# JingwenWang95/DSP-SLAM

Measured on NVIDIA H100. Metric: object-recons/sec (2048 pts, 10 GN iters), higher is better.
Workload: dtype f16x3-split (fp32 accumulate)

## Files before the change

### dsp_slam_b200/csrc/dspgn_api.cu

```cuda
#include <cuda_runtime.h>
#include <cstdio>
#include <cstring>
#include <cmath>
#include <string>
#include <vector>
#include <new>
#include <algorithm>
#include <atomic>

#include <cub/device/device_scan.cuh>

#include "dspgn_common.cuh"
#include "dspgn_simt.cuh"
#include "dspgn_solve.cuh"
#include "dspgn_tc.cuh"
#include "dspgn_mesh.cuh"
#include "dspgn_frame.cuh"
#include "dspgn_mono.cuh"

using namespace dspgn;

namespace {

constexpr int kEvCap = 1 << 18;
// ... 75 lines not shown
  DevBuf d_q_flag, d_q_ctr, d_tiles_left, d_obj_iter;
  int* d_tbase_static = nullptr;
  int* d_tbase_r_static = nullptr;
  DevBuf d_run;
  HostBuf h_run;
  cudaEvent_t ev_run_upload = nullptr;
  bool run_upload_pending = false;
  bool run_table_valid = false;
  bool run_table_gated = false;
  int total_tiles128 = 0;
  long long total_ray_tiles128 = 0;
  int max_tiles128 = 0;
  bool mega_enabled = true;
  bool compact_rays = true;
  DevBuf d_ev, d_seg, d_ln, d_vpre;
  bool events_on = false;
  HostBuf h_results;
  DspgnCounters ctr{};
  bool timing = false;
  std::vector<cudaEvent_t> ev;
  size_t ev_used = 0;
  std::vector<cudaEvent_t> ev_solve;
  size_t evs_used = 0;
  cudaEvent_t ev_run0 = nullptr, ev_run1 = nullptr;
  cudaStream_t stream2 = nullptr;
  cudaEvent_t ev_fork = nullptr, ev_join = nullptr;
  cudaEvent_t ev_upload = nullptr;
  bool upload_pending = false;
  bool mega_ran = false;
  bool band_rows_pending = false;
// ... 239 lines not shown
  int eng = cfg->engine;
  if (eng == DSPGN_ENGINE_AUTO) {
    const char* e = getenv("DSPGN_ENGINE");
    if (e && !strcmp(e, "simt")) eng = DSPGN_ENGINE_SIMT;
    else if (e && !strcmp(e, "tc")) eng = DSPGN_ENGINE_TC;
    else eng = (tc_ok && tc_engine_default()) ? DSPGN_ENGINE_TC : DSPGN_ENGINE_SIMT;
  }
  if (eng == DSPGN_ENGINE_TC && !tc_ok) { dspgn_solver_destroy(s); return fail(DSPGN_E_ARG, "tensor-core engine unavailable for this decoder shape"); }
  s->engine = eng;
  CU(cudaFuncSetAttribute(k_decoder_simt, cudaFuncAttributeMaxDynamicSharedMemorySize, (int)sizeof(SimtSmem)));
  for (auto* d : s->classes)
    if (d->has_ln) {
      if (s->d_ln.reserve(4 * (size_t)s->num_sms * DSPGN_MAX_LINEAR * kHid * kTP)) { dspgn_solver_destroy(s); return fail(DSPGN_E_ALLOC, "cudaMalloc"); }
      break;
    }
  if (int rc = tc_setup_kernels(g_err)) { dspgn_solver_destroy(s); return rc; }
  if (const char* m = getenv("DSPGN_MEGA")) s->mega_enabled = (m[0] != '0');
  if (const char* m = getenv("DSPGN_COMPACT_RAYS")) s->compact_rays = (m[0] != '0');
  if (cfg->schedule == DSPGN_SCHED_LAUNCHES) s->mega_enabled = false;
  else if (cfg->schedule == DSPGN_SCHED_PERSISTENT) s->mega_enabled = true;
  else if (cfg->schedule != DSPGN_SCHED_AUTO) { dspgn_solver_destroy(s); return fail(DSPGN_E_ARG, "bad schedule"); }
  s->events_on = getenv("DSPGN_CLK") != nullptr;
  CU(cudaEventCreateWithFlags(&s->ev_upload, cudaEventDisableTiming));
  CU(cudaEventCreateWithFlags(&s->ev_run_upload, cudaEventDisableTiming));
  CU(cudaStreamCreateWithFlags(&s->stream2, cudaStreamNonBlocking));
  CU(cudaEventCreateWithFlags(&s->ev_fork, cudaEventDisableTiming));
  CU(cudaEventCreateWithFlags(&s->ev_join, cudaEventDisableTiming));
  CU(cudaEventCreate(&s->ev_run0));
  CU(cudaEventCreate(&s->ev_run1));
#undef CU
// ... 3 lines not shown
    if (e_ != cudaSuccess)                                                                \
      return fail(DSPGN_E_CUDA, std::string(#call) + ": " + cudaGetErrorString(e_));      \
  } while (0)
  *out = s;
  return 0;
}

void dspgn_solver_destroy(DspgnSolver* s) {
  if (!s) return;
  cudaSetDevice(s->device);
  cudaDeviceSynchronize();
  s->flight.active = false;
  dspgn_gather_close(s);
  for (DevBuf* b : {&s->d_decs, &s->d_stage, &s->d_state, &s->d_part_s, &s->d_part_r, &s->d_tbase, &s->d_V, &s->d_m, &s->d_results, &s->d_active,
                    &s->d_sdf, &s->d_bx, &s->d_bs, &s->d_br, &s->d_dbg, &s->d_q_flag, &s->d_q_ctr,
                    &s->d_tiles_left, &s->d_obj_iter, &s->d_ev, &s->d_seg, &s->d_ln, &s->d_vpre, &s->d_run,
                    &s->d_grid_pts, &s->d_mgrid, &s->d_mws, &s->d_mscan_tmp, &s->d_mout, &s->d_mesh_sel}) b->release();
  s->h_stage.release();
  s->h_mbase.release();
  s->h_results.release();
  s->h_run.release();
  s->h_mesh_sel.release();
  s->h_flight.release();
  if (s->ev_flight) cudaEventDestroy(s->ev_flight);
  for (auto e : s->ev) cudaEventDestroy(e);
  for (auto e : s->ev_solve) cudaEventDestroy(e);
  if (s->ev_upload) cudaEventDestroy(s->ev_upload);
  if (s->ev_run_upload) cudaEventDestroy(s->ev_run_upload);
  if (s->ev_fork) cudaEventDestroy(s->ev_fork);
  if (s->ev_join) cudaEventDestroy(s->ev_join);
  if (s->stream2) cudaStreamDestroy(s->stream2);
// ... 426 lines not shown
    MegaArgs q;
    if (int rc = mega_args(s, p, q)) return rc;
    CU(cudaMemsetAsync(q.q_flag, 0, 4 * (size_t)q.q_cap, s->stream));
    if (int rc = launch_init(s, b, p, q)) return rc;
    TermArgs a = base_term(s, MODE_SDF);
    a.huber_b = s->cfg.b2;
    a.huber_b1 = s->cfg.b1;
    a.tile_base = s->d_tbase_static;
    a.part_r = s->d_part_r.as<float>(); a.tile_base_r = s->d_tbase_r_static;
    if (p.any[DSPGN_MODE_POSE] && p.iters[DSPGN_MODE_POSE] > 5) { a.pt_active = s->d_active.as<uint8_t>(); a.cut_iter = 4; }
    if (q.log.ev) CU(cudaMemsetAsync(q.log.ev, 0, 8, s->stream));
    SolveArgs v = base_solve(s);
    v.base_s = s->d_tbase_static; v.base_r = s->d_tbase_r_static; v.tile_rows = kTcRows; v.iter_index = 0;
    const int grid = grid_sms(s);
    if (s->timing) cudaEventRecord(next_event(s), s->stream);
    if (render) k_gn_persistent_render<<<grid, kTcThreads, kTcSmemBytes, s->stream>>>(b, a, q, v);
    else k_gn_persistent<<<grid, kTcThreads, kTcSmemBytes, s->stream>>>(b, a, q, v);
    if (s->timing) cudaEventRecord(next_event(s), s->stream);
    s->ctr.kernel_launches += 1;
    for (int m = 0; m < 2; ++m) s->ctr.rows_fwd_bwd += p.pts[m] * p.iters[m];
    s->band_rows_pending = render;
    s->mega_ran = true;
    CU(cudaGetLastError());
    CU(cudaEventRecord(s->ev_run1, s->stream));
    return 0;
  }
  if (int rc = launch_init(s, b, p)) return rc;
  auto iterate = [&](const RunPlan& pl, int n_iters) -> int {
    for (int e = 0; e < n_iters; ++e) {
      if (int rc = launch_terms(s, b, pl, e)) return rc;
      SolveArgs v = base_solve(s);
      v.iter_index = e;
// ... 1393 lines not shown
```

### dsp_slam_b200/csrc/dspgn_tc.cuh

```cuda
#pragma once
#include <cuda_fp16.h>
#include <string>
#include <vector>
#include "dspgn_simt.cuh"
#include "dspgn_solve.cuh"

namespace dspgn {

constexpr int kTcThreads = 384;
constexpr int kTcEpiThreads = 256;
constexpr int kTcStages = 4;
constexpr int kTcStageBytes = 16384;
constexpr int kTcAloBytes = 32768;
constexpr int kTcProducerRegs = 40, kTcConsumerRegs = 232;
static_assert(128 * kTcProducerRegs + 256 * kTcConsumerRegs <= 384 * 168, "setmaxnreg budget exceeds the CTA's registers");

__host__ __device__ constexpr int tc_mma_n(int n) { return n <= 80 ? 80 : (n <= 192 ? 192 : 256); }
__host__ __device__ constexpr int tc_pad_k_steps(int k_steps) { return (k_steps + 3) / 4 * 4; }

__device__ __forceinline__ uint32_t smem_u32(const void* p) { return (uint32_t)__cvta_generic_to_shared(p); }

__device__ __forceinline__ void mbar_init(uint64_t* bar, uint32_t count) {
  asm volatile("mbarrier.init.shared::cta.b64 [%0], %1;" ::"r"(smem_u32(bar)), "r"(count) : "memory");
}
__device__ __forceinline__ void mbar_arrive(uint32_t bar) {
  asm volatile("mbarrier.arrive.shared::cta.b64 _, [%0];" ::"r"(bar) : "memory");
}
// ... 6 lines not shown
      ".reg .pred p;\n\t"
      "WAIT_LOOP:\n\t"
      "mbarrier.try_wait.parity.shared::cta.b64 p, [%0], %1;\n\t"
      "@p bra DONE;\n\t"
      "bra WAIT_LOOP;\n\t"
      "DONE:\n\t"
      "}" ::"r"(bar), "r"(parity) : "memory");
}
__device__ __forceinline__ void mbar_wait(uint64_t* bar, uint32_t parity) { mbar_wait(smem_u32(bar), parity); }
__device__ __forceinline__ void fence_barrier_init() { asm volatile("fence.mbarrier_init.release.cluster;" ::: "memory"); }

__device__ __forceinline__ void bulk_g2s(void* smem_dst, const void* gmem_src, uint32_t bytes, uint64_t* bar) {
  asm volatile("cp.async.bulk.shared::cluster.global.mbarrier::complete_tx::bytes [%0], [%1], %2, [%3];" ::"r"(smem_u32(smem_dst)),
               "l"(gmem_src), "r"(bytes), "r"(smem_u32(bar)) : "memory");
}

__device__ __forceinline__ void fence_proxy_async() { asm volatile("fence.proxy.async.shared::cta;" ::: "memory"); }
__device__ __forceinline__ void wg_fence() { asm volatile("wgmma.fence.sync.aligned;" ::: "memory"); }
__device__ __forceinline__ void wg_commit() { asm volatile("wgmma.commit_group.sync.aligned;" ::: "memory"); }
__device__ __forceinline__ void wg_wait0() { asm volatile("wgmma.wait_group.sync.aligned 0;" ::: "memory"); }
__device__ __forceinline__ void wg_wait1() { asm volatile("wgmma.wait_group.sync.aligned 1;" ::: "memory"); }
template <int REGS> __device__ __forceinline__ void setmaxnreg_inc() { asm volatile("setmaxnreg.inc.sync.aligned.u32 %0;" ::"n"(REGS)); }
template <int REGS> __device__ __forceinline__ void setmaxnreg_dec() { asm volatile("setmaxnreg.dec.sync.aligned.u32 %0;" ::"n"(REGS)); }
__device__ __forceinline__ void wg_bar_sync(int g) { asm volatile("bar.sync %0, 128;" ::"r"(3 + g) : "memory"); }

#define DSPGN_D8(o) "+f"(d[o + 0]), "+f"(d[o + 1]), "+f"(d[o + 2]), "+f"(d[o + 3]), "+f"(d[o + 4]), "+f"(d[o + 5]), "+f"(d[o + 6]), "+f"(d[o + 7])
#define DSPGN_D128                                                                                                    \
  DSPGN_D8(0), DSPGN_D8(8), DSPGN_D8(16), DSPGN_D8(24), DSPGN_D8(32), DSPGN_D8(40), DSPGN_D8(48), DSPGN_D8(56),         \
      DSPGN_D8(64), DSPGN_D8(72), DSPGN_D8(80), DSPGN_D8(88), DSPGN_D8(96), DSPGN_D8(104), DSPGN_D8(112), DSPGN_D8(120)
#define DSPGN_D96                                                                                                     \
// ... 70 lines not shown
  d |= (uint64_t)1 << 16;
  d |= (uint64_t)32 << 32;
  d |= (uint64_t)2 << 62;
  return d;
}

__device__ __forceinline__ void split_pack(float a, float b, uint32_t& hi, uint32_t& lo) {
  __half2 h = __floats2half2_rn(a, b);
  float2 back = __half22float2(h);
  __half2 l = __floats2half2_rn(a - back.x, b - back.y);
  hi = *reinterpret_cast<uint32_t*>(&h);
  lo = *reinterpret_cast<uint32_t*>(&l);
}

constexpr int kJpStride = 76;
struct TcSmemTail {
  float Jp[kTcRows * kJpStride];
  uint32_t maskw[8 * 4 * kTcEpiThreads];
  float bias[9 * kHid];
  float wlast[kHid];
  float w0x[3 * kHid];
  float zs[kMaxCode + 16];
  float xr[3 * kTcRows];
  float rr[kTcRows], rsc[kTcRows];
  float yrow[kTcRows], scr[kTcRows];
  int prefix[kMaxObjScan + 1];
  int warp_tmp[32];
  uint64_t w_full[kTcStages], w_empty[kTcStages];
  int cur_class;
  int fifo[4]; int fifo_pub; int epi_seq; int last_flag;
  TcPlan plans[DSPGN_MAX_CLASSES];
  BatchDev ctx_b; MegaArgs ctx_q; SolveArgs ctx_sv;
  int push_base, push_nF, push_nS, push_o;
  float ost[16]; int ost_rows;
};
constexpr size_t kTcSmemBytes = 1024 + (size_t)kTcStages * kTcStageBytes + 2 * (size_t)kTcAloBytes + sizeof(TcSmemTail);
static_assert(kTcSmemBytes <= 227 * 1024, "tensor-core engine shared memory exceeds the 227 KB per block of sm_90");
static_assert(offsetof(TcSmemTail, bias) % 8 == 0 && offsetof(TcSmemTail, w0x) % 8 == 0,
              "the SDF-tile epilogues read bias and W0 column pairs as float2");

__device__ __forceinline__ int frag_col(int e, int q) { return 8 * (e >> 2) + 2 * q + (e & 1); }
__device__ __forceinline__ int opaque_int(int v) {
  int r;
  asm volatile("mov.b32 %0, %1;" : "=r"(r) : "r"(v));
  return r;
}

__device__ __forceinline__ void store_operand(const float (&v)[128], uint32_t (&ah)[64], unsigned char* alo, int rl, int q, int grp,
                                              int pslot = -1) {
  DSPGN_PROBE_T(ts);
#pragma unroll
  for (int t = 0; t < 16; ++t) {
#pragma unroll
    for (int h = 0; h < 4; ++h) {
// ... 146 lines not shown
      float w = hy ? bj.y : bj.x;
      w = fmaf(hy ? w0.y : w0.x, hb ? xb0 : xa0, w);
      w = fmaf(hy ? w1.y : w1.x, hb ? xb1 : xa1, w);
      w = fmaf(hy ? w2.y : w2.x, hb ? xb2 : xa2, w);
      mw[e >> 5] |= (w > 0.f ? 1u : 0u) << (e & 31);
      acc[e] = w > 0.f ? w : 0.f;
    }
  }
}

__device__ __forceinline__ void release_stage(uint32_t w_empty, int s) {
  __syncwarp();
  if ((threadIdx.x & 31) == 0) mbar_arrive(w_empty + 8u * s);
}

template <int N>
__device__ __forceinline__ void wg_gemm(float (&acc)[128], const uint32_t (&ah)[64], uint32_t alo, uint32_t ring,
                                        uint32_t bars, uint32_t& phase, int nch) {
  static_assert(kTcStages == 4, "one ring lap per K chunk");
  const uint32_t w_full = bars, w_empty = bars + 8u * kTcStages;
#pragma unroll
  for (int i = 0; i < 128; ++i) acc[i] = 0.f;
#pragma unroll
  for (int c = 0; c < 4; ++c) {
    if (c < nch) {
      const uint32_t ph = phase ^ (uint32_t)(c & 1);
#pragma unroll
      for (int s = 0; s < kTcStages; ++s) {
        DSPGN_PROBE_T(tf);
        mbar_wait(w_full + 8u * s, ph);
        DSPGN_PROBE_ADD(PR_WFULL, tf);
        wg_fence();
        const uint32_t bw = ring + (uint32_t)s * kTcStageBytes;
#pragma unroll
        for (int k = 0; k < 2; ++k) {
          const int t = 4 * c + 2 * (s & 1) + k;
          const uint64_t bd = make_desc_w(bw + 32u * k);
          Wgmma<N>::rs(acc, ah[4 * t], ah[4 * t + 1], ah[4 * t + 2], ah[4 * t + 3], bd);
          if (s < 2) Wgmma<N>::ss(acc, make_desc(alo + 8192u * c + 32u * (t & 3)), bd);
        }
        wg_commit();
        if (s == 1) {
          DSPGN_PROBE_T(tw);
          wg_wait1();
          DSPGN_PROBE_ADD(PR_WGWAIT, tw);
          release_stage(w_empty, 0);
          if (c > 0) release_stage(w_empty, 3);
        } else if (s == 3) {
          DSPGN_PROBE_T(tw);
          wg_wait1();
          DSPGN_PROBE_ADD(PR_WGWAIT, tw);
          release_stage(w_empty, 1);
          release_stage(w_empty, 2);
        }
      }
    }
  }
  DSPGN_PROBE_T(tw);
  wg_wait0();
  DSPGN_PROBE_ADD(PR_WGWAIT, tw);
  release_stage(w_empty, 3);
  phase ^= (uint32_t)(nch & 1);
}

__device__ __forceinline__ void produce_step(const unsigned char* src, int nch, uint32_t img_bytes, unsigned char* ring,
                                             uint64_t* w_full, uint64_t* w_empty, uint32_t& phase) {
  for (int c = 0; c < nch; ++c) {
    for (int s = 0; s < kTcStages; ++s) {
      DSPGN_PROBE_T(te);
      mbar_wait(&w_empty[s], phase ^ 1);
      DSPGN_PROBE_ADD(PR_WEMPTY, te);
      mbar_expect_tx(&w_full[s], img_bytes);
      bulk_g2s(ring + (size_t)s * kTcStageBytes, src + (size_t)(kTcStages * c + s) * img_bytes, img_bytes, &w_full[s]);
    }
    phase ^= 1;
  }
}

struct TileRef { int o, row0, slot, mode, tile; };

constexpr unsigned long long kMegaTimeoutNs = 30ull * 1000ull * 1000ull * 1000ull;
__device__ inline int mega_pop(const MegaArgs& q, int n_obj) {
  for (;;) {
    const int t = atomicAdd(&q.ctr->head, 1);
    if (t >= q.q_cap) return -1;
    unsigned long long t0 = 0;
    int item = kItemNop;
    for (unsigned spins = 0;; ++spins) {
      const int v = ldv(q.q_flag + t);
      if (v != 0) { __threadfence(); item = v - 1; break; }
      if (ldv(&q.ctr->done_objects) >= n_obj || ldv(&q.ctr->abort_flag) != 0) return -1;
      __nanosleep(256);
      if ((spins & 1023u) == 1023u) {
        const unsigned long long now = globaltimer_ns();
        if (t0 == 0) t0 = now;
        else if (now - t0 > kMegaTimeoutNs) { atomicExch(&q.ctr->abort_flag, 1); return -1; }
      }
    }
    if (item != kItemNop) return item;
  }
}

template <int SCHED>
__device__ __forceinline__ bool tile_at(const BatchDev& b, const TermArgs& a, TcSmemTail& S, int seq, int total_tiles, TileRef& t) {
  constexpr bool MEGA = SCHED != 0;
  if (!MEGA) {
    const int tile = blockIdx.x + seq * gridDim.x;
    if (tile >= total_tiles) return false;
    t.o = find_object(S.prefix, b.n_obj, tile);
    t.tile = tile - S.prefix[t.o];
    t.row0 = t.tile * kTcRows;
    t.slot = tile;
    t.mode = a.mode;
    return true;
  } else {
    volatile int* pub = &S.fifo_pub;
    while (*pub <= seq) __nanosleep(64);
    const int item = reinterpret_cast<volatile int*>(S.fifo)[seq & 3];
    if (item < 0) return false;
// ... 9 lines not shown

__device__ __forceinline__ int mega_rows(const BatchDev& b, const MegaArgs& q, const ObjMeta& M, int o, int mode) {
  if (mode == MODE_SDF) return M.n_pts;
  if (mode == MODE_BAND) return ldv(b.band_m + o);
  if (q.vpre != nullptr) return ldv(q.vpre + vpre_base(M, o) + M.n_rays) >> 7;
  return M.n_rays * b.D;
}

__device__ inline void mega_push(const MegaArgs& q, int kind, int o, int n) {
  if (n <= 0) return;
  const int base = atomicAdd(&q.ctr->tail, n);
  __threadfence();
  for (int j = 0; j < n; ++j) *reinterpret_cast<volatile int*>(q.q_flag + base + j) = make_item(kind, o, j) + 1;
}

__device__ __noinline__ void mega_solve_and_advance(TcSmemTail& S, int o, int tid) {
  const BatchDev& b = S.ctx_b;
  const MegaArgs& q = S.ctx_q;
  const SolveArgs& sv = S.ctx_sv;
  __threadfence();
  SolveSmem& SM = *reinterpret_cast<SolveSmem*>(S.Jp);
  const int it = ldv(q.obj_iter + o);
  const bool render = q.render && b.state[o].mode == DSPGN_MODE_JOINT;
  if (tid == 0) log_event(q.log, ev_desc(EV_SOLVE_BEGIN, 0, o, it));
  const int fin = solve_object<true>(b, sv, q.log, o, tid, SM, it + 1 >= b.state[o].n_iter);
  epi_bar_sync();
  int vh = -1;
  if (!fin && render && q.vpre != nullptr) {
    const ObjMeta M = b.meta[o];
    if (M.n_rays > 0) vh = valid_sample_ranges<true>(M, b.state[o], b.rays, b.D, q.vpre + vpre_base(M, o), tid, kTcEpiThreads, S.warp_tmp);
  }
// ... 23 lines not shown
    S.push_base = base;
  }
  epi_bar_sync();
  const int base = S.push_base;
  if (base >= 0) {
    const int nF = S.push_nF, n = nF + S.push_nS;
    const int po = S.push_o;
    __threadfence();
    epi_bar_sync();
    for (int j = tid; j < n; j += kTcEpiThreads)
      *reinterpret_cast<volatile int*>(q.q_flag + base + j) = ((j < nF) ? make_item(MODE_RAYFWD, po, j) : make_item(MODE_SDF, po, j - nF)) + 1;
  }
}

template <int SCHED>
__device__ __forceinline__ void tc_body(const BatchDev& b, const TermArgs& a, const MegaArgs& q, const SolveArgs& sv) {
  constexpr bool MEGA = SCHED != 0;
  constexpr bool RENDER = SCHED == 2;
  extern __shared__ unsigned char tc_smem_raw[];
  unsigned char* ring = tc_smem_raw + ((1024u - (smem_u32(tc_smem_raw) & 1023u)) & 1023u);
  TcSmemTail& S = *reinterpret_cast<TcSmemTail*>(ring + (size_t)kTcStages * kTcStageBytes + 2 * (size_t)kTcAloBytes);
  const int tid = threadIdx.x, warp = tid >> 5, lane = tid & 31;

  const int total_tiles = MEGA ? 0 : build_tile_prefix(b, a, kTcRows, S.prefix, S.warp_tmp);
  {
    const int nwords = b.n_classes * (int)(sizeof(TcPlan) / 4);
    for (int i = tid; i < nwords; i += kTcThreads) {
      const int c = i / (int)(sizeof(TcPlan) / 4), w = i % (int)(sizeof(TcPlan) / 4);
      reinterpret_cast<int*>(&S.plans[c])[w] = reinterpret_cast<const int*>(&b.decs[c].tc_plan)[w];
    }
  }
  if (tid == 0) {
    for (int i = 0; i < kTcStages; ++i) { mbar_init(&S.w_full[i], 1); mbar_init(&S.w_empty[i], 8); }
    S.cur_class = -1;
    S.fifo_pub = 0; S.epi_seq = 0; S.last_flag = 0;
    if (MEGA) { S.ctx_b = b; S.ctx_q = q; S.ctx_sv = sv; }
    fence_barrier_init();
  }
  __syncthreads();

  if (warp >= 8) {
    setmaxnreg_dec<kTcProducerRegs>();
    if (warp == 8 && lane == 0) {
      uint32_t phase = 0;
      DSPGN_PROBE_T(tloop);
      for (int seq = 0;; ++seq) {
        if (MEGA) {
          DSPGN_PROBE_T(tp);
          volatile int* es = &S.epi_seq;
          while (seq - *es >= 3) __nanosleep(64);
          const int item = mega_pop(q, b.n_obj);
          DSPGN_PROBE_ADD(PR_POP, tp);
          if (item >= 0) log_event(q.log, ev_desc(EV_POPPED, item >> kItemKindShift, (item >> kItemObjShift) & kItemObjMask, item & kItemTileMask));
          reinterpret_cast<volatile int*>(S.fifo)[seq & 3] = item;
          __threadfence_block();
          *reinterpret_cast<volatile int*>(&S.fifo_pub) = seq + 1;
        }
        TileRef tr;
        if (!tile_at<SCHED>(b, a, S, seq, total_tiles, tr)) break;
        const int o = tr.o;
        const int cls = b.meta[o].class_id;
        const TcPlan& plan = S.plans[cls];
        const unsigned char* blob = b.decs[cls].tc_blob;
        const bool fwd_only = (tr.mode == MODE_RAYFWD || tr.mode == MODE_PTSFWD || (!MEGA && tr.mode == MODE_GRIDFWD));
        const int ns = (RENDER && tr.mode == kKindScan) ? 0 : (fwd_only ? plan.n_fwd : plan.n_steps);
        for (int s = 0; s < ns; ++s)
          produce_step(blob + plan.step[s].w_off, plan.step[s].k_steps / 4, 64u * (uint32_t)plan.step[s].n_mma, ring, S.w_full,
                       S.w_empty, phase);
      }
      DSPGN_PROBE_ADD(PR_PROD_LOOP, tloop);
    }
  } else {
    setmaxnreg_inc<kTcConsumerRegs>();
    const int grp = warp >> 2;
    const int r = tid & 127;
    const int qd = lane & 3;
    const int rl = 16 * (warp & 3) + (lane >> 2);
    const int rowA = 64 * grp + rl, rowB = rowA + 8;
    unsigned char* const alo = ring + (size_t)kTcStages * kTcStageBytes + (size_t)grp * kTcAloBytes;
    const uint32_t alo_s = smem_u32(alo), ring_s = smem_u32(ring);
    uint32_t phase = 0;
    float acc[128];
    uint32_t ah[64];
    DSPGN_PROBE_T(tloop);
    for (int seq = 0;; ++seq) {
      TileRef tr;
      DSPGN_PROBE_T(tq);
      if (!tile_at<SCHED>(b, a, S, seq, total_tiles, tr)) break;
      DSPGN_PROBE_ADD(PR_FIFO, tq);
      DSPGN_PROBE_T(tpro);
      if (MEGA && tid == 0) { *reinterpret_cast<volatile int*>(&S.epi_seq) = seq + 1; log_event(q.log, ev_desc(EV_TILE_BEGIN, tr.mode, tr.o, tr.tile)); }
      if (RENDER && tr.mode == kKindScan) {
        const int o = tr.o;
        scan_chunk(b, sv.prm.th, q.vpre, q.seg_cnt, o, tr.tile, tid);
        __threadfence();
        epi_bar_sync();
// ... 109 lines not shown
          xform_point(Toc, __fmul_rn(rq[0], d), __fmul_rn(rq[1], d), __fmul_rn(rq[2], d), x0, x1, x2);
          sc = inside_unit_sphere(x0, x1, x2) ? 1.f : 0.f;
        }
      }
      if (grp == 0) { S.xr[r] = x0; S.xr[kTcRows + r] = x1; S.xr[2 * kTcRows + r] = x2; S.scr[r] = sc; }
      epi_bar_sync();
      DSPGN_PROBE_ADD(PR_PRO_GLOBAL, tpro);
      DSPGN_PROBE_T(tl0);
      if (tid == 0) S.cur_class = M.class_id;

      auto inp = [&](int i, int row) -> float {
        const int j = i - L;
        return (j < 0) ? S.zs[i] : ((unsigned)j < 3u ? S.xr[j * kTcRows + row] : 0.f);
      };
      uint32_t* const maskw = S.maskw + tid;
      auto put_operand = [&](int pslot) {
        if (SCHED == 1) store_operand_stsm(acc, ah, alo_s, grp, pslot);
        else store_operand(acc, ah, alo, rl, qd, grp, pslot);
      };

      {
        const int kk = plan.step[0].k_steps * 16;
        const int n0out = dec.out_dim[0];
        const float* w0x = S.w0x;
        const float xa0 = S.xr[rowA], xa1 = S.xr[kTcRows + rowA], xa2 = S.xr[2 * kTcRows + rowA];
        const float xb0 = S.xr[rowB], xb1 = S.xr[kTcRows + rowB], xb2 = S.xr[2 * kTcRows + rowB];
        const int qs = opaque_int(qd);
        uint32_t mw[4] = {0u, 0u, 0u, 0u};
        if (SCHED == 1 && kk == kHid && n0out == kHid) {
          epi_layer0_256(acc, mw, S.bias, w0x, qs, xa0, xa1, xa2, xb0, xb1, xb2);
        } else {
#pragma unroll
          for (int e = 0; e < 128; ++e) {
            const int c = frag_col(e, qs);
            const bool hb = (e & 2) != 0;
            float w = S.bias[c];
            w = fmaf(w0x[c], hb ? xb0 : xa0, w);
            w = fmaf(w0x[kHid + c], hb ? xb1 : xa1, w);
            w = fmaf(w0x[2 * kHid + c], hb ? xb2 : xa2, w);
            const bool on = (c < kk) && (c < n0out) && (w > 0.f);
            mw[e >> 5] |= (on ? 1u : 0u) << (e & 31);
            acc[e] = on ? w : 0.f;
          }
        }
#pragma unroll
        for (int w = 0; w < 4; ++w) maskw[w * kTcEpiThreads] = mw[w];
        put_operand(-1);
      }
      DSPGN_PROBE_ADD(PR_PRO_L0, tl0);
      DSPGN_PROBE_ADD(PR_PROLOGUE, tpro);
      DSPGN_PROBE_COUNT(PR_TILES);

      float yv = 0.f;
      for (int s = 0; s < ns; ++s) {
        const TcStep st = plan.step[s];
        const bool more = (s + 1 < ns);
        const int k_next = more ? plan.step[s + 1].k_steps * 16 : 0;
        const int nm = st.n_mma;
        if (MEGA && tid == 0 && s == 0) log_event(q.log, ev_desc(EV_FIRST_MMA, tr.mode, tr.o, tr.tile));
        const int nch = st.k_steps / 4;
        DSPGN_PROBE_T(tg);
        if (nm == 80) wg_gemm<80>(acc, ah, alo_s, ring_s, smem_u32(S.w_full), phase, nch);
        else if (nm == 192) wg_gemm<192>(acc, ah, alo_s, ring_s, smem_u32(S.w_full), phase, nch);
        else wg_gemm<256>(acc, ah, alo_s, ring_s, smem_u32(S.w_full), phase, nch);
        DSPGN_PROBE_ADD(PR_GEMM, tg);
        DSPGN_PROBE_T(tepi);
        wg_bar_sync(grp);
        DSPGN_PROBE_ADD(PR_EPI_ENTRY, tepi);
        DSPGN_PROBE_T(tval);
#ifdef DSPGN_STALL_PROBE
        const int pk = PR_EPI_KIND + 3 * (st.kind == TK_FWD_PENULT ? EK_PENULT
                                          : st.kind == TK_FWD_HIDDEN ? (st.cat_off >= 0 ? EK_FWD_CAT : EK_FWD)
                                          : st.kind == TK_BWD_MID ? (st.cat_off >= 0 ? EK_BWD_SKIP : EK_BWD) : EK_BWD_FIRST);
#else
        constexpr int pk = -1;
#endif
        const int qs = opaque_int(qd);

        if (st.kind == TK_FWD_PENULT) {
          const float* bb = S.bias + st.layer * kHid;
          float pa = 0.f, pb = 0.f;
          uint32_t mw[4] = {0u, 0u, 0u, 0u};
#pragma unroll
          for (int e = 0; e < 128; ++e) {
            const int c = frag_col(e, qs);
            if (c < nm) {
              const float w = acc[e] + bb[c];
              mw[e >> 5] |= (w > 0.f ? 1u : 0u) << (e & 31);
              if (e & 2) pb = fmaf(fmaxf(w, 0.f), S.wlast[c], pb);
              else pa = fmaf(fmaxf(w, 0.f), S.wlast[c], pa);
            }
          }
#pragma unroll
          for (int w = 0; w < 4; ++w) maskw[(4 * st.layer + w) * kTcEpiThreads] = mw[w];
          pa += __shfl_xor_sync(0xffffffffu, pa, 1);
          pb += __shfl_xor_sync(0xffffffffu, pb, 1);
          pa += __shfl_xor_sync(0xffffffffu, pa, 2);
          pb += __shfl_xor_sync(0xffffffffu, pb, 2);
          const float blast = S.bias[(st.layer + 1) * kHid];
          const float ya = tanhf(pa + blast), yb = tanhf(pb + blast);
          if (qd == 0) { S.yrow[rowA] = ya; S.yrow[rowB] = yb; }
          epi_bar_sync();
          yv = S.yrow[r];
          if (fwd_only) {
            if (grp == 0 && r < nrows) {
              const size_t base = (mode == MODE_RAYFWD) ? (size_t)M.smp_off
                                  : (grid_mode ? (size_t)a.grid_slot[o] * a.grid_rows : (size_t)M.pts_off);
              b.sdf[base + row0 + r] = (sc != 0.f) ? yv : INFINITY;
            }
// ... 25 lines not shown
            else if (st.cat_off >= 0) epi_concat_input<0, 0>(acc, qs, k_next, st.cat_off, L, S.zs, S.xr, rowA, rowB);
          } else {
#pragma unroll
            for (int e = 0; e < 128; ++e) {
              const int c = frag_col(e, qs);
              float t = 0.f;
              if (c < nm) {
                const float w = acc[e] + bb[c];
                mw[e >> 5] |= (w > 0.f ? 1u : 0u) << (e & 31);
                t = fmaxf(w, 0.f);
              }
              if (st.cat_off >= 0 && c >= st.cat_off) t = inp(c - st.cat_off, (e & 2) ? rowB : rowA);
              acc[e] = (c < k_next) ? t : 0.f;
            }
          }
#pragma unroll
          for (int w = 0; w < 4; ++w) maskw[(4 * st.layer + w) * kTcEpiThreads] = mw[w];
          DSPGN_PROBE_ADD(pk, tval);
          put_operand(pk);
        } else if (st.kind == TK_BWD_MID) {
          uint32_t mw[4];
#pragma unroll
          for (int w = 0; w < 4; ++w) mw[w] = maskw[(4 * st.mask_layer + w) * kTcEpiThreads];
          if (SCHED == 1) {
            if (st.cat_off == 189 && L == 64 && in0 == 67 && nm == kHid) epi_skip_grad<189, 64>(acc, qs, nm, st.cat_off, in0, L, S.Jp, rowA, rowB);
            else if (st.cat_off >= 0) epi_skip_grad<0, 0>(acc, qs, nm, st.cat_off, in0, L, S.Jp, rowA, rowB);
            if (nm == 256 && k_next == 256) epi_bwd_mid<256, 256>(acc, mw, nm, k_next);
            else if (nm == 256 && k_next == 192) epi_bwd_mid<256, 192>(acc, mw, nm, k_next);
            else epi_bwd_mid<0, 0>(acc, mw, nm, k_next);
          } else {
#pragma unroll
            for (int e = 0; e < 128; ++e) {
              const int c = frag_col(e, qs);
              float t = 0.f;
              if (c < nm) {
                const float v = acc[e];
                t = ((mw[e >> 5] >> (e & 31)) & 1u) ? v : 0.f;
                if (st.cat_off >= 0 && c >= st.cat_off) {
// ... 141 lines not shown
        }
        DSPGN_PROBE_ADD(PR_TILE_END, tend);
        if (act == 2) {
          DSPGN_PROBE_T(tsv);
          mega_solve_and_advance(S, o, tid);
          DSPGN_PROBE_ADD(PR_SOLVE, tsv);
          DSPGN_PROBE_COUNT(PR_SOLVES);
        }
      }
    }
    DSPGN_PROBE_ADD(PR_LOOP, tloop);
  }
}

__global__ void __launch_bounds__(kTcThreads, 1) k_decoder_tc(BatchDev b, TermArgs a) {
  tc_body<0>(b, a, MegaArgs{}, SolveArgs{});
}
__global__ void __launch_bounds__(kTcThreads, 1) k_gn_persistent(BatchDev b, TermArgs a, MegaArgs q, SolveArgs sv) {
  tc_body<1>(b, a, q, sv);
}
__global__ void __launch_bounds__(kTcThreads, 1) k_gn_persistent_render(BatchDev b, TermArgs a, MegaArgs q, SolveArgs sv) {
  tc_body<2>(b, a, q, sv);
}

constexpr size_t kTcSelftestSmem = 1024 + (size_t)kTcStages * kTcStageBytes + 2 * (size_t)kTcAloBytes + 64;
__global__ void __launch_bounds__(kTcThreads, 1) k_tc_selftest(const float* __restrict__ A, int lda, const unsigned char* __restrict__ blob,
                                                               int n_mma, int k_steps, float* __restrict__ D) {
  extern __shared__ unsigned char st_raw[];
  unsigned char* ring = st_raw + ((1024u - (smem_u32(st_raw) & 1023u)) & 1023u);
  uint64_t* bars = reinterpret_cast<uint64_t*>(ring + (size_t)kTcStages * kTcStageBytes + 2 * (size_t)kTcAloBytes);
  uint64_t* w_full = bars;
  uint64_t* w_empty = bars + kTcStages;
  const int tid = threadIdx.x, warp = tid >> 5, lane = tid & 31;
  if (tid == 0) {
    for (int i = 0; i < kTcStages; ++i) { mbar_init(&w_full[i], 1); mbar_init(&w_empty[i], 8); }
    fence_barrier_init();
  }
  __syncthreads();
  const int n_img = tc_mma_n(n_mma), nch = tc_pad_k_steps(k_steps) / 4;
  uint32_t phase = 0;
  if (warp >= 8) {
    setmaxnreg_dec<kTcProducerRegs>();
    if (warp == 8 && lane == 0) produce_step(blob, nch, 64u * (uint32_t)n_img, ring, w_full, w_empty, phase);
    return;
  }
  setmaxnreg_inc<kTcConsumerRegs>();
  const int grp = warp >> 2, qd = lane & 3, rl = 16 * (warp & 3) + (lane >> 2);
  const int rowA = 64 * grp + rl, rowB = rowA + 8;
  unsigned char* alo = ring + (size_t)kTcStages * kTcStageBytes + (size_t)grp * kTcAloBytes;
  float acc[128];
  uint32_t ah[64];
#pragma unroll
  for (int e = 0; e < 128; ++e) {
    const int c = frag_col(e, qd);
    acc[e] = (c < k_steps * 16) ? A[(size_t)((e & 2) ? rowB : rowA) * lda + c] : 0.f;
  }
  store_operand(acc, ah, alo, rl, qd, grp);
  if (n_img == 80) wg_gemm<80>(acc, ah, smem_u32(alo), smem_u32(ring), smem_u32(bars), phase, nch);
  else if (n_img == 192) wg_gemm<192>(acc, ah, smem_u32(alo), smem_u32(ring), smem_u32(bars), phase, nch);
  else wg_gemm<256>(acc, ah, smem_u32(alo), smem_u32(ring), smem_u32(bars), phase, nch);
#pragma unroll
  for (int e = 0; e < 128; ++e) {
    const int c = frag_col(e, qd);
    if (c < n_mma) D[(size_t)((e & 2) ? rowB : rowA) * n_mma + c] = acc[e];
  }
}

struct TcDecoderHost {
  bool ok = false;
  void* blob = nullptr;
  size_t blob_bytes = 0;
};

template <class F>
inline void tc_pack_images(std::vector<unsigned char>& out, int n_img, int k_steps, F&& elem) {
// ... 68 lines not shown
  P.n_steps = ns;
  void* d = nullptr;
  if (cudaMalloc(&d, blob.size()) != cudaSuccess) { cudaGetLastError(); err = "cudaMalloc(tc blob)"; return DSPGN_E_ALLOC; }
  if (cudaMemcpy(d, blob.data(), blob.size(), cudaMemcpyHostToDevice) != cudaSuccess) { cudaFree(d); err = "cudaMemcpy(tc blob)"; return DSPGN_E_CUDA; }
  h.blob = d; h.blob_bytes = blob.size(); h.ok = true;
  dv->tc_blob = reinterpret_cast<const unsigned char*>(d);
  return 0;
}

inline void tc_free_decoder(TcDecoderHost& h) {
  if (h.blob) cudaFree(h.blob);
  h.blob = nullptr; h.ok = false;
}

inline int tc_setup_kernels(std::string& err) {
  if (cudaFuncSetAttribute(k_decoder_tc, cudaFuncAttributeMaxDynamicSharedMemorySize, (int)kTcSmemBytes) != cudaSuccess) {
    err = std::string("cudaFuncSetAttribute(k_decoder_tc): ") + cudaGetErrorString(cudaGetLastError());
    return DSPGN_E_CUDA;
  }
  if (cudaFuncSetAttribute(k_gn_persistent, cudaFuncAttributeMaxDynamicSharedMemorySize, (int)kTcSmemBytes) != cudaSuccess ||
      cudaFuncSetAttribute(k_gn_persistent_render, cudaFuncAttributeMaxDynamicSharedMemorySize, (int)kTcSmemBytes) != cudaSuccess) {
    err = std::string("cudaFuncSetAttribute(k_gn_persistent): ") + cudaGetErrorString(cudaGetLastError());
    return DSPGN_E_CUDA;
  }
  if (cudaFuncSetAttribute(k_tc_selftest, cudaFuncAttributeMaxDynamicSharedMemorySize, (int)kTcSelftestSmem) != cudaSuccess) {
    err = std::string("cudaFuncSetAttribute(k_tc_selftest): ") + cudaGetErrorString(cudaGetLastError());
    return DSPGN_E_CUDA;
  }
  return 0;
}

inline bool tc_engine_default() { return true; }

inline int tc_launch_term(const BatchDev& b, const TermArgs& a, int num_sms, long long tiles_upper, cudaStream_t stream,
                          std::string& err) {
  int grid = (int)std::min<long long>(tiles_upper, num_sms);
  if (grid < 1) grid = 1;
  k_decoder_tc<<<grid, kTcThreads, kTcSmemBytes, stream>>>(b, a);
  (void)err;
  return 0;
}

}
```

Measured before the change: 5376.

## Deepen persistent kernel weight ring by spilling ReLU masks to global memory

In the persistent Gauss-Newton kernel, the per-layer ReLU masks are written to a per-block global buffer instead of an 8-layer shared-memory array. During backward passes they are prefetched with cp.async into a single-layer smem slot. The prefix scan array also shrinks to one element. The freed shared memory grows the weight-streaming TMA ring from 4 to 6 stages, so the ring now tracks a rolling slot and phase. The goal is deeper prefetch of weight images ahead of wgmma, at the cost of extra global mask traffic and more complex ring indexing.

```diff
diff --git a/dsp_slam_b200/csrc/dspgn_api.cu b/dsp_slam_b200/csrc/dspgn_api.cu
--- a/dsp_slam_b200/csrc/dspgn_api.cu
+++ b/dsp_slam_b200/csrc/dspgn_api.cu
@@ -113,6 +113,7 @@
   bool mega_enabled = true;
   bool compact_rays = true;
   DevBuf d_ev, d_seg, d_ln, d_vpre;
+  DevBuf d_masks;
   bool events_on = false;
   HostBuf h_results;
   DspgnCounters ctr{};
@@ -382,6 +383,8 @@
       if (s->d_ln.reserve(4 * (size_t)s->num_sms * DSPGN_MAX_LINEAR * kHid * kTP)) { dspgn_solver_destroy(s); return fail(DSPGN_E_ALLOC, "cudaMalloc"); }
       break;
     }
+  if (eng == DSPGN_ENGINE_TC &&
+      s->d_masks.reserve(sizeof(uint4) * (size_t)s->num_sms * kTcMaskLayers * kTcEpiThreads)) { dspgn_solver_destroy(s); return fail(DSPGN_E_ALLOC, "cudaMalloc"); }
   if (int rc = tc_setup_kernels(g_err)) { dspgn_solver_destroy(s); return rc; }
   if (const char* m = getenv("DSPGN_MEGA")) s->mega_enabled = (m[0] != '0');
   if (const char* m = getenv("DSPGN_COMPACT_RAYS")) s->compact_rays = (m[0] != '0');
@@ -415,7 +418,7 @@
   dspgn_gather_close(s);
   for (DevBuf* b : {&s->d_decs, &s->d_stage, &s->d_state, &s->d_part_s, &s->d_part_r, &s->d_tbase, &s->d_V, &s->d_m, &s->d_results, &s->d_active,
                     &s->d_sdf, &s->d_bx, &s->d_bs, &s->d_br, &s->d_dbg, &s->d_q_flag, &s->d_q_ctr,
-                    &s->d_tiles_left, &s->d_obj_iter, &s->d_ev, &s->d_seg, &s->d_ln, &s->d_vpre, &s->d_run,
+                    &s->d_tiles_left, &s->d_obj_iter, &s->d_ev, &s->d_seg, &s->d_ln, &s->d_vpre, &s->d_masks, &s->d_run,
                     &s->d_grid_pts, &s->d_mgrid, &s->d_mws, &s->d_mscan_tmp, &s->d_mout, &s->d_mesh_sel}) b->release();
   s->h_stage.release();
   s->h_mbase.release();
@@ -872,8 +875,8 @@
     v.base_s = s->d_tbase_static; v.base_r = s->d_tbase_r_static; v.tile_rows = kTcRows; v.iter_index = 0;
     const int grid = grid_sms(s);
     if (s->timing) cudaEventRecord(next_event(s), s->stream);
-    if (render) k_gn_persistent_render<<<grid, kTcThreads, kTcSmemBytes, s->stream>>>(b, a, q, v);
-    else k_gn_persistent<<<grid, kTcThreads, kTcSmemBytes, s->stream>>>(b, a, q, v);
+    if (render) k_gn_persistent_render<<<grid, kTcThreads, kTcSmemBytes<2>, s->stream>>>(b, a, q, v);
+    else k_gn_persistent<<<grid, kTcThreads, kTcSmemBytes<1>, s->stream>>>(b, a, q, v, s->d_masks.as<uint4>());
     if (s->timing) cudaEventRecord(next_event(s), s->stream);
     s->ctr.kernel_launches += 1;
     for (int m = 0; m < 2; ++m) s->ctr.rows_fwd_bwd += p.pts[m] * p.iters[m];
diff --git a/dsp_slam_b200/csrc/dspgn_tc.cuh b/dsp_slam_b200/csrc/dspgn_tc.cuh
--- a/dsp_slam_b200/csrc/dspgn_tc.cuh
+++ b/dsp_slam_b200/csrc/dspgn_tc.cuh
@@ -11,6 +11,7 @@
 constexpr int kTcEpiThreads = 256;
 constexpr int kTcStages = 4;
 constexpr int kTcStageBytes = 16384;
+template <int SCHED> constexpr int kTcRing = SCHED == 1 ? 6 : kTcStages;
 constexpr int kTcAloBytes = 32768;
 constexpr int kTcProducerRegs = 40, kTcConsumerRegs = 232;
 static_assert(128 * kTcProducerRegs + 256 * kTcConsumerRegs <= 384 * 168, "setmaxnreg budget exceeds the CTA's registers");
@@ -47,6 +48,11 @@
   asm volatile("cp.async.bulk.shared::cluster.global.mbarrier::complete_tx::bytes [%0], [%1], %2, [%3];" ::"r"(smem_u32(smem_dst)),
                "l"(gmem_src), "r"(bytes), "r"(smem_u32(bar)) : "memory");
 }
+
+__device__ __forceinline__ void cp_async_16(uint32_t smem_dst, const void* gmem_src) {
+  asm volatile("cp.async.cg.shared.global [%0], [%1], 16;" ::"r"(smem_dst), "l"(gmem_src) : "memory");
+}
+__device__ __forceinline__ void cp_async_wait_all() { asm volatile("cp.async.wait_all;" ::: "memory"); }
 
 __device__ __forceinline__ void fence_proxy_async() { asm volatile("fence.proxy.async.shared::cta;" ::: "memory"); }
 __device__ __forceinline__ void wg_fence() { asm volatile("wgmma.fence.sync.aligned;" ::: "memory"); }
@@ -147,9 +153,11 @@
 }
 
 constexpr int kJpStride = 76;
+constexpr int kTcMaskLayers = 8;
+template <int SCHED>
 struct TcSmemTail {
   float Jp[kTcRows * kJpStride];
-  uint32_t maskw[8 * 4 * kTcEpiThreads];
+  uint32_t maskw[(SCHED == 1 ? 1 : kTcMaskLayers) * 4 * kTcEpiThreads];
   float bias[9 * kHid];
   float wlast[kHid];
   float w0x[3 * kHid];
@@ -157,9 +165,9 @@
   float xr[3 * kTcRows];
   float rr[kTcRows], rsc[kTcRows];
   float yrow[kTcRows], scr[kTcRows];
-  int prefix[kMaxObjScan + 1];
+  int prefix[SCHED == 1 ? 1 : kMaxObjScan + 1];
   int warp_tmp[32];
-  uint64_t w_full[kTcStages], w_empty[kTcStages];
+  uint64_t w_full[kTcRing<SCHED>], w_empty[kTcRing<SCHED>];
   int cur_class;
   int fifo[4]; int fifo_pub; int epi_seq; int last_flag;
   TcPlan plans[DSPGN_MAX_CLASSES];
@@ -167,10 +175,14 @@
   int push_base, push_nF, push_nS, push_o;
   float ost[16]; int ost_rows;
 };
-constexpr size_t kTcSmemBytes = 1024 + (size_t)kTcStages * kTcStageBytes + 2 * (size_t)kTcAloBytes + sizeof(TcSmemTail);
-static_assert(kTcSmemBytes <= 227 * 1024, "tensor-core engine shared memory exceeds the 227 KB per block of sm_90");
-static_assert(offsetof(TcSmemTail, bias) % 8 == 0 && offsetof(TcSmemTail, w0x) % 8 == 0,
+template <int SCHED>
+constexpr size_t kTcSmemBytes = 1024 + (size_t)kTcRing<SCHED> * kTcStageBytes + 2 * (size_t)kTcAloBytes + sizeof(TcSmemTail<SCHED>);
+static_assert(kTcSmemBytes<0> <= 227 * 1024, "k_decoder_tc: shared memory exceeds the 227 KB per block of sm_90");
+static_assert(kTcSmemBytes<1> <= 227 * 1024, "k_gn_persistent: shared memory exceeds the 227 KB per block of sm_90");
+static_assert(kTcSmemBytes<2> <= 227 * 1024, "k_gn_persistent_render: shared memory exceeds the 227 KB per block of sm_90");
+static_assert(offsetof(TcSmemTail<1>, bias) % 8 == 0 && offsetof(TcSmemTail<1>, w0x) % 8 == 0,
               "the SDF-tile epilogues read bias and W0 column pairs as float2");
+static_assert(offsetof(TcSmemTail<1>, maskw) % 16 == 0, "the SDF-tile kernel stages one uint4 of masks per thread");
 
 __device__ __forceinline__ int frag_col(int e, int q) { return 8 * (e >> 2) + 2 * q + (e & 1); }
 __device__ __forceinline__ int opaque_int(int v) {
@@ -347,24 +359,34 @@
   if ((threadIdx.x & 31) == 0) mbar_arrive(w_empty + 8u * s);
 }
 
-template <int N>
+template <int RING>
+__device__ __forceinline__ void ring_at(uint32_t stage, uint32_t phase, uint32_t k, uint32_t& slot, uint32_t& par) {
+  const uint32_t g = stage + k, laps = g / RING;
+  slot = g - RING * laps;
+  par = phase ^ (laps & 1u);
+}
+
+template <int N, int RING>
 __device__ __forceinline__ void wg_gemm(float (&acc)[128], const uint32_t (&ah)[64], uint32_t alo, uint32_t ring,
-                                        uint32_t bars, uint32_t& phase, int nch) {
-  static_assert(kTcStages == 4, "one ring lap per K chunk");
-  const uint32_t w_full = bars, w_empty = bars + 8u * kTcStages;
+                                        uint32_t bars, uint32_t& stage, uint32_t& phase, int nch) {
+  static_assert(RING >= kTcStages, "the ring holds at least one K chunk");
+  const uint32_t w_full = bars, w_empty = bars + 8u * RING;
+  const uint32_t st0 = (RING == kTcStages) ? 0u : stage;
+  auto slot_of = [&](int k) { uint32_t sl, p; ring_at<RING>(st0, phase, (uint32_t)k, sl, p); return sl; };
 #pragma unroll
   for (int i = 0; i < 128; ++i) acc[i] = 0.f;
 #pragma unroll
   for (int c = 0; c < 4; ++c) {
     if (c < nch) {
-      const uint32_t ph = phase ^ (uint32_t)(c & 1);
 #pragma unroll
       for (int s = 0; s < kTcStages; ++s) {
+        uint32_t slot, ph;
+        ring_at<RING>(st0, phase, (uint32_t)(kTcStages * c + s), slot, ph);
         DSPGN_PROBE_T(tf);
-        mbar_wait(w_full + 8u * s, ph);
+        mbar_wait(w_full + 8u * slot, ph);
         DSPGN_PROBE_ADD(PR_WFULL, tf);
         wg_fence();
-        const uint32_t bw = ring + (uint32_t)s * kTcStageBytes;
+        const uint32_t bw = ring + slot * kTcStageBytes;
 #pragma unroll
         for (int k = 0; k < 2; ++k) {
           const int t = 4 * c + 2 * (s & 1) + k;
@@ -377,14 +399,14 @@
           DSPGN_PROBE_T(tw);
           wg_wait1();
           DSPGN_PROBE_ADD(PR_WGWAIT, tw);
-          release_stage(w_empty, 0);
-          if (c > 0) release_stage(w_empty, 3);
+          release_stage(w_empty, slot_of(kTcStages * c));
+          if (c > 0) release_stage(w_empty, slot_of(kTcStages * c - 1));
         } else if (s == 3) {
           DSPGN_PROBE_T(tw);
           wg_wait1();
           DSPGN_PROBE_ADD(PR_WGWAIT, tw);
-          release_stage(w_empty, 1);
-          release_stage(w_empty, 2);
+          release_stage(w_empty, slot_of(kTcStages * c + 1));
+          release_stage(w_empty, slot_of(kTcStages * c + 2));
         }
       }
     }
@@ -392,22 +414,27 @@
   DSPGN_PROBE_T(tw);
   wg_wait0();
   DSPGN_PROBE_ADD(PR_WGWAIT, tw);
-  release_stage(w_empty, 3);
-  phase ^= (uint32_t)(nch & 1);
-}
-
+  release_stage(w_empty, slot_of(kTcStages * nch - 1));
+  ring_at<RING>(st0, phase, (uint32_t)(kTcStages * nch), stage, phase);
+}
+
+template <int RING>
 __device__ __forceinline__ void produce_step(const unsigned char* src, int nch, uint32_t img_bytes, unsigned char* ring,
-                                             uint64_t* w_full, uint64_t* w_empty, uint32_t& phase) {
+                                             uint64_t* w_full, uint64_t* w_empty, uint32_t& stage, uint32_t& phase) {
+  uint32_t st = (RING == kTcStages) ? 0u : stage;
   for (int c = 0; c < nch; ++c) {
     for (int s = 0; s < kTcStages; ++s) {
+      uint32_t slot, ph;
+      ring_at<RING>(st, phase, (uint32_t)s, slot, ph);
       DSPGN_PROBE_T(te);
-      mbar_wait(&w_empty[s], phase ^ 1);
+      mbar_wait(&w_empty[slot], ph ^ 1);
       DSPGN_PROBE_ADD(PR_WEMPTY, te);
-      mbar_expect_tx(&w_full[s], img_bytes);
-      bulk_g2s(ring + (size_t)s * kTcStageBytes, src + (size_t)(kTcStages * c + s) * img_bytes, img_bytes, &w_full[s]);
-    }
-    phase ^= 1;
-  }
+      mbar_expect_tx(&w_full[slot], img_bytes);
+      bulk_g2s(ring + (size_t)slot * kTcStageBytes, src + (size_t)(kTcStages * c + s) * img_bytes, img_bytes, &w_full[slot]);
+    }
+    ring_at<RING>(st, phase, (uint32_t)kTcStages, st, phase);
+  }
+  stage = st;
 }
 
 struct TileRef { int o, row0, slot, mode, tile; };
@@ -435,7 +462,7 @@
 }
 
 template <int SCHED>
-__device__ __forceinline__ bool tile_at(const BatchDev& b, const TermArgs& a, TcSmemTail& S, int seq, int total_tiles, TileRef& t) {
+__device__ __forceinline__ bool tile_at(const BatchDev& b, const TermArgs& a, TcSmemTail<SCHED>& S, int seq, int total_tiles, TileRef& t) {
   constexpr bool MEGA = SCHED != 0;
   if (!MEGA) {
     const int tile = blockIdx.x + seq * gridDim.x;
@@ -475,7 +502,8 @@
   for (int j = 0; j < n; ++j) *reinterpret_cast<volatile int*>(q.q_flag + base + j) = make_item(kind, o, j) + 1;
 }
 
-__device__ __noinline__ void mega_solve_and_advance(TcSmemTail& S, int o, int tid) {
+template <int SCHED>
+__device__ __noinline__ void mega_solve_and_advance(TcSmemTail<SCHED>& S, int o, int tid) {
   const BatchDev& b = S.ctx_b;
   const MegaArgs& q = S.ctx_q;
   const SolveArgs& sv = S.ctx_sv;
@@ -529,12 +557,14 @@
 }
 
 template <int SCHED>
-__device__ __forceinline__ void tc_body(const BatchDev& b, const TermArgs& a, const MegaArgs& q, const SolveArgs& sv) {
+__device__ __forceinline__ void tc_body(const BatchDev& b, const TermArgs& a, const MegaArgs& q, const SolveArgs& sv,
+                                        uint4* __restrict__ masks_g) {
   constexpr bool MEGA = SCHED != 0;
   constexpr bool RENDER = SCHED == 2;
+  constexpr int RING = kTcRing<SCHED>;
   extern __shared__ unsigned char tc_smem_raw[];
   unsigned char* ring = tc_smem_raw + ((1024u - (smem_u32(tc_smem_raw) & 1023u)) & 1023u);
-  TcSmemTail& S = *reinterpret_cast<TcSmemTail*>(ring + (size_t)kTcStages * kTcStageBytes + 2 * (size_t)kTcAloBytes);
+  TcSmemTail<SCHED>& S = *reinterpret_cast<TcSmemTail<SCHED>*>(ring + (size_t)RING * kTcStageBytes + 2 * (size_t)kTcAloBytes);
   const int tid = threadIdx.x, warp = tid >> 5, lane = tid & 31;
 
   const int total_tiles = MEGA ? 0 : build_tile_prefix(b, a, kTcRows, S.prefix, S.warp_tmp);
@@ -546,7 +576,7 @@
     }
   }
   if (tid == 0) {
-    for (int i = 0; i < kTcStages; ++i) { mbar_init(&S.w_full[i], 1); mbar_init(&S.w_empty[i], 8); }
+    for (int i = 0; i < RING; ++i) { mbar_init(&S.w_full[i], 1); mbar_init(&S.w_empty[i], 8); }
     S.cur_class = -1;
     S.fifo_pub = 0; S.epi_seq = 0; S.last_flag = 0;
     if (MEGA) { S.ctx_b = b; S.ctx_q = q; S.ctx_sv = sv; }
@@ -557,7 +587,7 @@
   if (warp >= 8) {
     setmaxnreg_dec<kTcProducerRegs>();
     if (warp == 8 && lane == 0) {
-      uint32_t phase = 0;
+      uint32_t stage = 0, phase = 0;
       DSPGN_PROBE_T(tloop);
       for (int seq = 0;; ++seq) {
         if (MEGA) {
@@ -580,8 +610,8 @@
         const bool fwd_only = (tr.mode == MODE_RAYFWD || tr.mode == MODE_PTSFWD || (!MEGA && tr.mode == MODE_GRIDFWD));
         const int ns = (RENDER && tr.mode == kKindScan) ? 0 : (fwd_only ? plan.n_fwd : plan.n_steps);
         for (int s = 0; s < ns; ++s)
-          produce_step(blob + plan.step[s].w_off, plan.step[s].k_steps / 4, 64u * (uint32_t)plan.step[s].n_mma, ring, S.w_full,
-                       S.w_empty, phase);
+          produce_step<RING>(blob + plan.step[s].w_off, plan.step[s].k_steps / 4, 64u * (uint32_t)plan.step[s].n_mma, ring,
+                             S.w_full, S.w_empty, stage, phase);
       }
       DSPGN_PROBE_ADD(PR_PROD_LOOP, tloop);
     }
@@ -592,9 +622,9 @@
     const int qd = lane & 3;
     const int rl = 16 * (warp & 3) + (lane >> 2);
     const int rowA = 64 * grp + rl, rowB = rowA + 8;
-    unsigned char* const alo = ring + (size_t)kTcStages * kTcStageBytes + (size_t)grp * kTcAloBytes;
+    unsigned char* const alo = ring + (size_t)RING * kTcStageBytes + (size_t)grp * kTcAloBytes;
     const uint32_t alo_s = smem_u32(alo), ring_s = smem_u32(ring);
-    uint32_t phase = 0;
+    uint32_t stage = 0, phase = 0;
     float acc[128];
     uint32_t ah[64];
     DSPGN_PROBE_T(tloop);
@@ -734,6 +764,15 @@
         return (j < 0) ? S.zs[i] : ((unsigned)j < 3u ? S.xr[j * kTcRows + row] : 0.f);
       };
       uint32_t* const maskw = S.maskw + tid;
+      auto mask_g = [&](int l) { return masks_g + ((size_t)blockIdx.x * kTcMaskLayers + l) * kTcEpiThreads + tid; };
+      auto save_mask = [&](int l, const uint32_t (&mw)[4]) {
+        if (SCHED == 1) {
+          *mask_g(l) = make_uint4(mw[0], mw[1], mw[2], mw[3]);
+        } else {
+#pragma unroll
+          for (int w = 0; w < 4; ++w) maskw[(4 * l + w) * kTcEpiThreads] = mw[w];
+        }
+      };
       auto put_operand = [&](int pslot) {
         if (SCHED == 1) store_operand_stsm(acc, ah, alo_s, grp, pslot);
         else store_operand(acc, ah, alo, rl, qd, grp, pslot);
@@ -763,8 +802,7 @@
             acc[e] = on ? w : 0.f;
           }
         }
-#pragma unroll
-        for (int w = 0; w < 4; ++w) maskw[w * kTcEpiThreads] = mw[w];
+        save_mask(0, mw);
         put_operand(-1);
       }
       DSPGN_PROBE_ADD(PR_PRO_L0, tl0);
@@ -779,10 +817,11 @@
         const int nm = st.n_mma;
         if (MEGA && tid == 0 && s == 0) log_event(q.log, ev_desc(EV_FIRST_MMA, tr.mode, tr.o, tr.tile));
         const int nch = st.k_steps / 4;
+        if (SCHED == 1 && st.kind == TK_BWD_MID) cp_async_16(smem_u32(S.maskw) + 16u * (uint32_t)tid, mask_g(st.mask_layer));
         DSPGN_PROBE_T(tg);
-        if (nm == 80) wg_gemm<80>(acc, ah, alo_s, ring_s, smem_u32(S.w_full), phase, nch);
-        else if (nm == 192) wg_gemm<192>(acc, ah, alo_s, ring_s, smem_u32(S.w_full), phase, nch);
-        else wg_gemm<256>(acc, ah, alo_s, ring_s, smem_u32(S.w_full), phase, nch);
+        if (nm == 80) wg_gemm<80, RING>(acc, ah, alo_s, ring_s, smem_u32(S.w_full), stage, phase, nch);
+        else if (nm == 192) wg_gemm<192, RING>(acc, ah, alo_s, ring_s, smem_u32(S.w_full), stage, phase, nch);
+        else wg_gemm<256, RING>(acc, ah, alo_s, ring_s, smem_u32(S.w_full), stage, phase, nch);
         DSPGN_PROBE_ADD(PR_GEMM, tg);
         DSPGN_PROBE_T(tepi);
         wg_bar_sync(grp);
@@ -811,8 +850,7 @@
               else pa = fmaf(fmaxf(w, 0.f), S.wlast[c], pa);
             }
           }
-#pragma unroll
-          for (int w = 0; w < 4; ++w) maskw[(4 * st.layer + w) * kTcEpiThreads] = mw[w];
+          save_mask(st.layer, mw);
           pa += __shfl_xor_sync(0xffffffffu, pa, 1);
           pb += __shfl_xor_sync(0xffffffffu, pb, 1);
           pa += __shfl_xor_sync(0xffffffffu, pa, 2);
@@ -868,14 +906,19 @@
               acc[e] = (c < k_next) ? t : 0.f;
             }
           }
-#pragma unroll
-          for (int w = 0; w < 4; ++w) maskw[(4 * st.layer + w) * kTcEpiThreads] = mw[w];
+          save_mask(st.layer, mw);
           DSPGN_PROBE_ADD(pk, tval);
           put_operand(pk);
         } else if (st.kind == TK_BWD_MID) {
           uint32_t mw[4];
-#pragma unroll
-          for (int w = 0; w < 4; ++w) mw[w] = maskw[(4 * st.mask_layer + w) * kTcEpiThreads];
+          if (SCHED == 1) {
+            cp_async_wait_all();
+            const uint4 m = reinterpret_cast<const uint4*>(S.maskw)[tid];
+            mw[0] = m.x; mw[1] = m.y; mw[2] = m.z; mw[3] = m.w;
+          } else {
+#pragma unroll
+            for (int w = 0; w < 4; ++w) mw[w] = maskw[(4 * st.mask_layer + w) * kTcEpiThreads];
+          }
           if (SCHED == 1) {
             if (st.cat_off == 189 && L == 64 && in0 == 67 && nm == kHid) epi_skip_grad<189, 64>(acc, qs, nm, st.cat_off, in0, L, S.Jp, rowA, rowB);
             else if (st.cat_off >= 0) epi_skip_grad<0, 0>(acc, qs, nm, st.cat_off, in0, L, S.Jp, rowA, rowB);
@@ -1047,13 +1090,13 @@
 }
 
 __global__ void __launch_bounds__(kTcThreads, 1) k_decoder_tc(BatchDev b, TermArgs a) {
-  tc_body<0>(b, a, MegaArgs{}, SolveArgs{});
-}
-__global__ void __launch_bounds__(kTcThreads, 1) k_gn_persistent(BatchDev b, TermArgs a, MegaArgs q, SolveArgs sv) {
-  tc_body<1>(b, a, q, sv);
+  tc_body<0>(b, a, MegaArgs{}, SolveArgs{}, nullptr);
+}
+__global__ void __launch_bounds__(kTcThreads, 1) k_gn_persistent(BatchDev b, TermArgs a, MegaArgs q, SolveArgs sv, uint4* masks) {
+  tc_body<1>(b, a, q, sv, masks);
 }
 __global__ void __launch_bounds__(kTcThreads, 1) k_gn_persistent_render(BatchDev b, TermArgs a, MegaArgs q, SolveArgs sv) {
-  tc_body<2>(b, a, q, sv);
+  tc_body<2>(b, a, q, sv, nullptr);
 }
 
 constexpr size_t kTcSelftestSmem = 1024 + (size_t)kTcStages * kTcStageBytes + 2 * (size_t)kTcAloBytes + 64;
@@ -1071,10 +1114,10 @@
   }
   __syncthreads();
   const int n_img = tc_mma_n(n_mma), nch = tc_pad_k_steps(k_steps) / 4;
-  uint32_t phase = 0;
+  uint32_t stage = 0, phase = 0;
   if (warp >= 8) {
     setmaxnreg_dec<kTcProducerRegs>();
-    if (warp == 8 && lane == 0) produce_step(blob, nch, 64u * (uint32_t)n_img, ring, w_full, w_empty, phase);
+    if (warp == 8 && lane == 0) produce_step<kTcStages>(blob, nch, 64u * (uint32_t)n_img, ring, w_full, w_empty, stage, phase);
     return;
   }
   setmaxnreg_inc<kTcConsumerRegs>();
@@ -1089,9 +1132,9 @@
     acc[e] = (c < k_steps * 16) ? A[(size_t)((e & 2) ? rowB : rowA) * lda + c] : 0.f;
   }
   store_operand(acc, ah, alo, rl, qd, grp);
-  if (n_img == 80) wg_gemm<80>(acc, ah, smem_u32(alo), smem_u32(ring), smem_u32(bars), phase, nch);
-  else if (n_img == 192) wg_gemm<192>(acc, ah, smem_u32(alo), smem_u32(ring), smem_u32(bars), phase, nch);
-  else wg_gemm<256>(acc, ah, smem_u32(alo), smem_u32(ring), smem_u32(bars), phase, nch);
+  if (n_img == 80) wg_gemm<80, kTcStages>(acc, ah, smem_u32(alo), smem_u32(ring), smem_u32(bars), stage, phase, nch);
+  else if (n_img == 192) wg_gemm<192, kTcStages>(acc, ah, smem_u32(alo), smem_u32(ring), smem_u32(bars), stage, phase, nch);
+  else wg_gemm<256, kTcStages>(acc, ah, smem_u32(alo), smem_u32(ring), smem_u32(bars), stage, phase, nch);
 #pragma unroll
   for (int e = 0; e < 128; ++e) {
     const int c = frag_col(e, qd);
@@ -1190,12 +1233,12 @@
 }
 
 inline int tc_setup_kernels(std::string& err) {
-  if (cudaFuncSetAttribute(k_decoder_tc, cudaFuncAttributeMaxDynamicSharedMemorySize, (int)kTcSmemBytes) != cudaSuccess) {
+  if (cudaFuncSetAttribute(k_decoder_tc, cudaFuncAttributeMaxDynamicSharedMemorySize, (int)kTcSmemBytes<0>) != cudaSuccess) {
     err = std::string("cudaFuncSetAttribute(k_decoder_tc): ") + cudaGetErrorString(cudaGetLastError());
     return DSPGN_E_CUDA;
   }
-  if (cudaFuncSetAttribute(k_gn_persistent, cudaFuncAttributeMaxDynamicSharedMemorySize, (int)kTcSmemBytes) != cudaSuccess ||
-      cudaFuncSetAttribute(k_gn_persistent_render, cudaFuncAttributeMaxDynamicSharedMemorySize, (int)kTcSmemBytes) != cudaSuccess) {
+  if (cudaFuncSetAttribute(k_gn_persistent, cudaFuncAttributeMaxDynamicSharedMemorySize, (int)kTcSmemBytes<1>) != cudaSuccess ||
+      cudaFuncSetAttribute(k_gn_persistent_render, cudaFuncAttributeMaxDynamicSharedMemorySize, (int)kTcSmemBytes<2>) != cudaSuccess) {
     err = std::string("cudaFuncSetAttribute(k_gn_persistent): ") + cudaGetErrorString(cudaGetLastError());
     return DSPGN_E_CUDA;
   }
@@ -1212,7 +1255,7 @@
                           std::string& err) {
   int grid = (int)std::min<long long>(tiles_upper, num_sms);
   if (grid < 1) grid = 1;
-  k_decoder_tc<<<grid, kTcThreads, kTcSmemBytes, stream>>>(b, a);
+  k_decoder_tc<<<grid, kTcThreads, kTcSmemBytes<0>, stream>>>(b, a);
   (void)err;
   return 0;
 }
```

Result: faster. 5554, median of 6 (+3.3%).
